# PRADUMAN-KR/Multimodal-Lip-Sync-Deepfake-Detection-System

Measured on NVIDIA B200. Metric: windows_per_sec, higher is better.
Workload: dtype bf16

## Files before the change

### multimodal-lip-sync-deepfake-detection-system_b200/csrc/bf16_path.cu

```cuda
#include "forward_common.h"
#include "tok_front.cuh"
#include "tok_fused.cuh"
#include "token_kernels.cuh"
#include "umma_conv.cuh"
#include "stem_ring.cuh"

#include <cuda_fp16.h>

#include <algorithm>
#include <array>
#include <cstdio>
#include <cstdlib>
#include <cstring>
#include <functional>

using namespace lsd;
using namespace lsdfw;

#define LSD_ENV(name) ([]() -> const char* { static const char* const v_ = getenv(name); return v_; }())

namespace {

uint16_t f2bf(float f) {
  uint32_t u;
// ... 653 lines not shown
        const long long cy = d[3] - d[2];
        cmin = std::min(cmin, cy); cmax = std::max(cmax, cy); csum += cy;
      }
      fprintf(stderr, "[sr] %d CTAs x %d steps: kernel span %.1f us (globaltimer), latest CTA start +%.1f us, CTA cycles min %lld avg %lld max %lld\n", nc,
              p.nsteps, (g1 - g0) / 1e3, smax / 1e3, cmin, csum / nc, cmax);
    }
    const long long t0 = hv[0];
    for (int k = 0; k < 32; ++k)
      fprintf(stderr, "[sr] step %2d | prod free %7lld issued %7lld | mma landed %7lld blockfree %7lld issued %7lld | epi complete %7lld back %7lld\n", k + 16,
              hv[(0 * 32 + k) * 2] - t0, hv[(0 * 32 + k) * 2 + 1] - t0, hv[(1 * 32 + k) * 2] - t0, hv[(1 * 32 + k) * 2 + 1] - t0,
              hv[(2 * 32 + k) * 2] - t0, hv[(3 * 32 + k) * 2] - t0, hv[(3 * 32 + k) * 2 + 1] - t0);
    h->prof.end(c.st);
    return 0;
  }
  launch_stem_ring(p, tab->grid, c.st);
  h->prof.end(c.st);
  return 0;
}

#define RUN(name, ...)                            \
  do {                                            \
    UArgs a_;                                     \
    __VA_ARGS__;                                  \
    if ((rc = run_umma(b, name, a_))) return rc;  \
  } while (0)

#define RUNC(ctx, name, ...)                        \
  do {                                              \
    UArgs a_;                                       \
    __VA_ARGS__;                                    \
    if ((rc = run_umma(ctx, name, a_))) return rc;  \
  } while (0)

#define RUNS(name, ...)                            \
  do {                                             \
    UArgs a_;                                      \
    __VA_ARGS__;                                   \
    if ((rc = run_umma(bs, name, a_))) return rc;  \
  } while (0)

PlanarOut pout(const BCtx& c, const PBuf& p, const PBuf* lo = nullptr, int plane_off = 0) {
  PlanarOut o;
  o.y = c.org(p) + (int64_t)plane_off * p.plane_stride;
  o.ylo = lo ? c.org(*lo) + (int64_t)plane_off * lo->plane_stride : nullptr;
  o.plane_stride = p.plane_stride;
  if (p.g.ow > 0 && p.g.HP == 1) { o.grp = p.g.W; o.grp_stride = p.g.RW; o.off = p.g.ow; }
  else { o.grp = 0; o.grp_stride = 0; o.off = 0; }
  return o;
}

int res_stage_umma(const BCtx& b, const std::string& p, const PBuf& x, const PBuf& mid, const PBuf& y, bool has_ds, int y_mode,
                   const PBuf* x_lo = nullptr, const PBuf* mid_lo = nullptr, const PBuf* y_lo = nullptr) {
  int rc = 0;
  RUN(p + ".conv1", a_.in = &x; a_.in_lo = x_lo; a_.og = mid.g; a_.act = ACT_RELU; a_.yp = &mid; a_.yp_lo = mid_lo);
  if (has_ds) RUN(p + ".conv2", a_.in = &mid; a_.in_lo = mid_lo; a_.in_ds = &x; a_.in_ds_lo = x_lo; a_.og = mid.g; a_.act = ACT_RELU;
                  a_.yp = &y; a_.yp_lo = y_lo; a_.y_mode = y_mode);
  else RUN(p + ".conv2", a_.in = &mid; a_.in_lo = mid_lo; a_.og = mid.g; a_.act = ACT_RELU; a_.yp = &y; a_.yp_lo = y_lo; a_.y_mode = y_mode;
           a_.res = &x; a_.res_lo = x_lo);
  return 0;
}

int run_umma_fold(const BCtx& c, const std::string& name, const PBuf& x, int Hi, int Wi, int stride, const PBuf* x_ds, int Hd, int Wd,
                  int Ho, int Wo, const PBuf& yp, int y_mode) {
  const auto itL = c.h->blayers.find(name + "#fold");
  if (itL == c.h->blayers.end()) return lsd_fail(c.h, LSD_ERR_UNSUPPORTED, "%s: no weights packed for the folded route (LSD_FOLD=0)", name.c_str());
  const BLayer& L = itL->second;
  const UcGeom& og = x.g;
  if (og.P_total >= ((int64_t)1 << 31) - 1024) return lsd_fail(c.h, LSD_ERR_SHAPE, "%s: more than 2^31 rows in one launch (reduce the batch)", name.c_str());
  if ((L.groups.size() == 2) != (x_ds != nullptr) || x.sets != Hi * Wi || (x_ds && x_ds->sets != Hd * Wd))
    return lsd_fail(c.h, LSD_ERR_ARG, "%s: folded inputs do not match the layer", name.c_str());
  UmmaConvP p;
  memset(&p, 0, sizeof(p));
  p.w = reinterpret_cast<const __nv_bfloat16*>(c.h->barena);
  p.bias = c.h->bbias + L.bias_off;
  p.Cout = L.ntile;
  p.act = ACT_RELU;
  p.g = og;
  p.fold = 1;
  p.y_mode = y_mode;
  p.y = c.org(yp);
  p.y_plane_stride = yp.plane_stride; p.y_set_stride = yp.set_stride;
  p.g2 = yp.g;
  p.ymap_W = Wo;
  int mt = 2;
  if (const char* e = LSD_ENV("LSD_FOLD_MT")) mt = std::max(1, std::min(4, atoi(e)));
  p.MT = (int)std::max<int64_t>(1, std::min<int64_t>(mt, (og.P_total + 127) / 128));
  p.nbuf = 1;
  p.issuers = std::min(p.MT, 4);
  uint32_t cols = 32;
  while ((int)cols < p.MT * L.ntile) cols *= 2;
  p.tmem_cols = cols;
  const int S = p.MT * 128;
  const PBuf* srcs[2] = {&x, x_ds};
  p.ngroups = (int)L.groups.size();
  p.nbands = p.ngroups;
  int max_a = 0, max_w = 0, min_k16 = 1 << 30;
  for (int gi = 0; gi < p.ngroups; ++gi) {
    const BGroup& G = L.groups[gi];
    UcGroup& ug = p.groups[gi];
    ug.band_begin = gi; ug.band_end = gi + 1;
    ug.k16 = G.k16; ug.taps_total = G.taps_total;
    ug.w_off = (int64_t)G.w_off; ug.slice_stride = (int64_t)G.slice_stride;
    UcBand& ub = p.bands[gi];
    const PBuf& src = *srcs[gi];
    ub.base = c.org(src);
    ub.plane_stride = src.plane_stride;
    ub.chunk_stride = 2 * src.plane_stride;
    ub.ntaps = gi == 0 ? 3 : 1;
    ub.start = gi == 0 ? -1 : 0;
    ub.len_extra = gi == 0 ? 2 : 0;
    for (int j = 0; j < ub.ntaps; ++j) ub.rel[j] = j;
    if ((int64_t)8 > src.origin) return lsd_fail(c.h, LSD_ERR_UNSUPPORTED, "%s: guard zone too small", name.c_str());
    max_a = std::max(max_a, 2 * (S + ub.len_extra) * 16);
    max_w = std::max(max_w, ub.ntaps * L.ntile * 32);
    min_k16 = std::min(min_k16, G.k16);
  }
  p.kpack = std::max(1, std::min(std::min(8, min_k16), (48 * 1024) / (max_a + max_w)));
  p.a_stage_bytes = ((uint32_t)(max_a * p.kpack) + 127u) & ~127u;
  p.w_stage_bytes = (uint32_t)(max_w * p.kpack);
  const int cslices = L.Cout / L.ntile;
  std::vector<std::array<int, 3>> pos;
  auto inb = [&](int o, int k, int n) { const int i = stride * o + k - 1; return i >= 0 && i < n; };
  for (int ho = 0; ho < Ho; ++ho)
    for (int wo = 0; wo < Wo; ++wo) {
      int nq = 0;
      for (int kh = 0; kh < 3; ++kh)
        for (int kw = 0; kw < 3; ++kw) nq += inb(ho, kh, Hi) && inb(wo, kw, Wi);
      pos.push_back({-nq, ho, wo});
    }
  std::stable_sort(pos.begin(), pos.end(), [](const std::array<int, 3>& a, const std::array<int, 3>& b) { return a[0] < b[0]; });
  const int nslices = (int)pos.size() * cslices;
  if (nslices > UC_MAX_FSLICES || Ho > 255 || Wo > 255) return lsd_fail(c.h, LSD_ERR_UNSUPPORTED, "%s: map too large for the folded route", name.c_str());
  auto chunks = [&](int k16) { return (k16 + p.kpack - 1) / p.kpack; };
  int off = 0;
  for (int i = 0; i < nslices; ++i) {
    const auto& q = pos[(size_t)(i / cslices)];
    const int nst = -q[0] * chunks(p.groups[0].k16) + (x_ds ? chunks(p.groups[1].k16) : 0);
    p.fslice[i] = UcFoldSlice{(uint16_t)off, (uint16_t)nst, (uint8_t)q[1], (uint8_t)q[2], (uint8_t)(i % cslices), 0};
    p.nst_tile = std::max(p.nst_tile, nst);
    off += nst;
  }
  if (off > 65535) return lsd_fail(c.h, LSD_ERR_UNSUPPORTED, "%s: folded stage programs too long", name.c_str());
  const uint32_t stage = p.a_stage_bytes + p.w_stage_bytes;
  const uint32_t prog_bytes = (uint32_t)p.nst_tile * (uint32_t)umma_conv_stage_desc_bytes();
  const uint32_t budget = 211u * 1024u - (uint32_t)umma_conv_extra_smem_bytes(p);
  if (prog_bytes + 2 * stage > budget) return lsd_fail(c.h, LSD_ERR_UNSUPPORTED, "%s: stage program of %u bytes does not fit", name.c_str(), prog_bytes);
  p.stages = std::max(2, std::min((int)((budget - prog_bytes) / stage), 8));
  if (const char* e = getenv("LSD_UMMA_SKIP")) p.skip = atoi(e);
  if (const char* why = umma_conv_config_error(p)) return lsd_fail(c.h, LSD_ERR_UNSUPPORTED, "%s: %s", name.c_str(), why);
  auto build = [&](std::vector<UcStageDesc>& v) {
    for (int i = 0; i < nslices; ++i) {
      const UcFoldSlice& f = p.fslice[i];
      for (int kh = 0; kh < 3; ++kh)
        for (int kw = 0; kw < 3; ++kw) {
          if (!inb(f.h, kh, Hi) || !inb(f.w, kw, Wi)) continue;
          UcBand bq = p.bands[0];
          bq.base = c.org(x) + (int64_t)((stride * f.h + kh - 1) * Wi + stride * f.w + kw - 1) * x.set_stride;
          bq.tap_begin = (kh * 3 + kw) * 3;
          for (int c0 = 0; c0 < p.groups[0].k16; c0 += p.kpack) v.push_back(umma_conv_stage(p, p.groups[0], bq, 0, c0, f.col));
        }
      if (x_ds) {
        UcBand bd = p.bands[1];
        bd.base = c.org(*x_ds) + (int64_t)(2 * f.h * Wd + 2 * f.w) * x_ds->set_stride;
        for (int c0 = 0; c0 < p.groups[1].k16; c0 += p.kpack) v.push_back(umma_conv_stage(p, p.groups[1], bd, 1, c0, f.col));
      }
    }
  };
  if (int rc = stage_program(c, name + "#fold", p, build, {(uint64_t)Hi, (uint64_t)Wi, (uint64_t)stride, (uint64_t)Hd, (uint64_t)Wd,
                                                          (uint64_t)x.set_stride, (uint64_t)(x_ds ? x_ds->set_stride : 0)})) return rc;
  double kflop = 0;
  for (const BGroup& G : L.groups) kflop += (double)G.taps_total * G.Cin;
  c.h->prof.begin(c.st, 2.0 * (double)og.N * og.T * Ho * Wo * L.Cout * kflop, 2);
  launch_umma_conv(p, nslices, c.st, c.h->num_sms, c.max_ctas);
  c.h->prof.end(c.st);
  return 0;
}

int res_stage_fold(const BCtx& b, const std::string& p, const PBuf& x, int Hi, int Wi, const PBuf& mid, int Ho, int Wo, const PBuf& y, int y_mode) {
  int rc = 0;
  if ((rc = run_umma_fold(b, p + ".conv1", x, Hi, Wi, 2, nullptr, 0, 0, Ho, Wo, mid, UC_Y_FOLD))) return rc;
  return run_umma_fold(b, p + ".conv2", mid, Ho, Wo, 1, &x, Hi, Wi, Ho, Wo, y, y_mode);
}

}

static int pack_tok_fused(lsd_handle* h, const std::vector<float>& f32) {
  std::vector<TfBlock> blocks;
  tf_layer_blocks(blocks);
  std::vector<uint32_t> stage_bytes;
  for (const TfBlock& b : blocks)
    for (int k0 = 0; k0 < b.k16; k0 += b.kps) stage_bytes.push_back((uint32_t)b.kps * (uint32_t)b.N * 32u);
  std::vector<__half> w;
  std::vector<float> vec((size_t)TF_LAYERS * TF_VEC_LAYER + (size_t)(2 * TF_LAYERS + 1) * TF_D, 0.f);
  std::vector<float> cum(TF_D, 0.f);
  float* cum_out = vec.data() + (size_t)TF_LAYERS * TF_VEC_LAYER;
  for (int l = 0; l < TF_LAYERS; ++l) {
    const std::string k = "t" + std::to_string(l);
    const ConvP &cin = h->convs.at(k + ".in"), &cout = h->convs.at(k + ".out"), &cf1 = h->convs.at(k + ".ff1"), &cf2 = h->convs.at(k + ".ff2");
    const size_t w0 = w.size();
    for (const TfBlock& b : blocks) {
      const ConvP& c = b.kind == 0 ? cin : (b.kind == 1 ? cout : (b.kind == 2 ? cf1 : cf2));
      for (int k16 = 0; k16 < b.k16; ++k16)
        for (int pl = 0; pl < 2; ++pl)
          for (int n = 0; n < b.N; ++n)
            for (int e = 0; e < 8; ++e) {
              const int kk = k16 * 16 + pl * 8 + e;
              int co, ci;
              if (b.kind == 0) { co = ((n % 96) / 32) * 256 + (2 * b.idx + n / 96) * 32 + (n % 32); ci = kk; }
              else if (b.kind == 1) { co = n; ci = 64 * b.idx + kk; }
              else if (b.kind == 2) { co = 128 * b.idx + n; ci = kk; }
              else { co = n; ci = 128 * b.idx + kk; }
              w.push_back(__float2half_rn(f32[c.w_off + (size_t)ci * c.Cout + co]));
            }
    }
    if (l == 0) h->tokf_layer_bytes = (uint32_t)((w.size() - w0) * sizeof(__half));
    float* lv = vec.data() + (size_t)l * TF_VEC_LAYER;
    const char* names[4] = {".ln1.w", ".ln1.b", ".ln2.w", ".ln2.b"};
    for (int i = 0; i < 4; ++i) memcpy(lv + 256 * i, &f32[h->vecs.at(k + names[i])], 256 * sizeof(float));
    for (int n = 0; n < 768; ++n) {
      const int hp = n / 192, r = n % 192;
      lv[1024 + n] = f32[cin.shift_off + ((r % 96) / 32) * 256 + (2 * hp + r / 96) * 32 + (r % 32)];
    }
    memcpy(lv + 1024 + 768, &f32[cf1.shift_off], 1024 * sizeof(float));
    memcpy(cum_out + (size_t)(2 * l) * TF_D, cum.data(), TF_D * sizeof(float));
    for (int i = 0; i < TF_D; ++i) cum[i] += f32[cout.shift_off + i];
    memcpy(cum_out + (size_t)(2 * l + 1) * TF_D, cum.data(), TF_D * sizeof(float));
    for (int i = 0; i < TF_D; ++i) cum[i] += f32[cf2.shift_off + i];
  }
  memcpy(cum_out + (size_t)(2 * TF_LAYERS) * TF_D, cum.data(), TF_D * sizeof(float));
  h->tokf_n_stage = (int)stage_bytes.size();
  for (void* q : {(void*)h->tokf_w, (void*)h->tokf_stage_bytes, (void*)h->tokf_vec}) if (q) cudaFree(q);
  h->tokf_w = nullptr; h->tokf_stage_bytes = nullptr; h->tokf_vec = nullptr;
  cudaError_t e = cudaMalloc(&h->tokf_w, w.size() * sizeof(__half));
  if (e == cudaSuccess) e = cudaMemcpy(h->tokf_w, w.data(), w.size() * sizeof(__half), cudaMemcpyHostToDevice);
  if (e == cudaSuccess) e = cudaMalloc(&h->tokf_stage_bytes, stage_bytes.size() * sizeof(uint32_t));
  if (e == cudaSuccess) e = cudaMemcpy(h->tokf_stage_bytes, stage_bytes.data(), stage_bytes.size() * sizeof(uint32_t), cudaMemcpyHostToDevice);
  if (e == cudaSuccess) e = cudaMalloc(&h->tokf_vec, vec.size() * sizeof(float));
  if (e == cudaSuccess) e = cudaMemcpy(h->tokf_vec, vec.data(), vec.size() * sizeof(float), cudaMemcpyHostToDevice);
  if (e != cudaSuccess) return lsd_fail(h, LSD_ERR_CUDA, "pack_tok_fused: %s", cudaGetErrorString(e));
  return 0;
}

static int pack_tok_front(lsd_handle* h, const std::vector<float>& f32) {
  std::vector<__half> w;
  w.reserve((size_t)TFR_K16_TOTAL * 16 * 256);
  auto emit = [&](int k16, auto&& get) {
    for (int k = 0; k < k16; ++k)
      for (int pl = 0; pl < 2; ++pl)
        for (int n = 0; n < 256; ++n)
          for (int e = 0; e < 8; ++e) w.push_back(__float2half_rn(get(k * 16 + pl * 8 + e, n)));
  };
  const ConvP &o0 = h->convs.at("cross.v2a.out"), &o1 = h->convs.at("cross.a2v.out"), &g0 = h->convs.at("cross.gate0"),
// ... 732 lines not shown
```

### multimodal-lip-sync-deepfake-detection-system_b200/csrc/umma_conv.cu

```cuda
#include "umma_conv.cuh"
#include "token_kernels.cuh"

#include <algorithm>
#include <cstdio>
#include <cstdlib>
#include <cstring>

#include "lsd_kernels.h"
#include "umma.cuh"

namespace lsd {

using namespace umma;

struct F8 { float v[8]; };
__device__ __noinline__ F8 gelu8(F8 x) {
#pragma unroll
  for (int e = 0; e < 8; ++e) x.v[e] = 0.5f * x.v[e] * (1.0f + erff(x.v[e] * 0.70710678118654752f));
  return x;
}

__device__ __forceinline__ float uc_act(float v, int act) {
  if (act == ACT_RELU) return fmaxf(v, 0.0f);
  if (act == ACT_GELU) return 0.5f * v * (1.0f + erff(v * 0.70710678118654752f));
// ... 334 lines not shown
              for (int q = 0; q < 4; ++q) pre[4 + q] = *reinterpret_cast<const uint4*>(p.res_lo + roff + (int64_t)q * p.res_plane_stride);
            }
          } else if (use_r32) {
#pragma unroll
            for (int q = 0; q < 8; ++q) pre[q] = *reinterpret_cast<const uint4*>(r32row + c0 + 4 * q);
          }
          tmem_ld_wait();
#pragma unroll
          for (int q = 0; q < 4; ++q) {
            const int c = c0 + 8 * q;
            F8 x;
#pragma unroll
            for (int e = 0; e < 8; ++e) x.v[e] = v[8 * q + e];
            if (valid) {
              const float4 b0 = *reinterpret_cast<const float4*>(&bias_s[c]);
              const float4 b1 = *reinterpret_cast<const float4*>(&bias_s[c + 4]);
              x.v[0] += b0.x; x.v[1] += b0.y; x.v[2] += b0.z; x.v[3] += b0.w; x.v[4] += b1.x; x.v[5] += b1.y; x.v[6] += b1.z; x.v[7] += b1.w;
              if (use_res) {
                float f[8];
                unpack8(pre[q], f);
#pragma unroll
                for (int e = 0; e < 8; ++e) x.v[e] += f[e];
                if (use_lo) {
                  unpack8(pre[4 + q], f);
#pragma unroll
                  for (int e = 0; e < 8; ++e) x.v[e] += f[e];
                }
              } else if (use_r32) {
                const uint4 q0 = pre[2 * q], q1 = pre[2 * q + 1];
                x.v[0] += __uint_as_float(q0.x); x.v[1] += __uint_as_float(q0.y); x.v[2] += __uint_as_float(q0.z); x.v[3] += __uint_as_float(q0.w);
                x.v[4] += __uint_as_float(q1.x); x.v[5] += __uint_as_float(q1.y); x.v[6] += __uint_as_float(q1.z); x.v[7] += __uint_as_float(q1.w);
              }
              if (p.act == ACT_GELU) {
                x = gelu8(x);
              } else {
#pragma unroll
                for (int e = 0; e < 8; ++e) x.v[e] = fmaxf(x.v[e], act_lo);
              }
              if (y32row) {
                float4* o = reinterpret_cast<float4*>(y32row + c);
                o[0] = make_float4(x.v[0], x.v[1], x.v[2], x.v[3]);
                o[1] = make_float4(x.v[4], x.v[5], x.v[6], x.v[7]);
              }
            } else {
#pragma unroll
              for (int e = 0; e < 8; ++e) x.v[e] = 0.0f;
            }
            if (store_planar) {
              const uint4 hi4 = pack8(x.v);
              const int64_t off = (int64_t)((ch0 + c) >> 3) * p.y_plane_stride + dst;
              *reinterpret_cast<uint4*>(p.y + off) = hi4;
              if (p.ylo) {
                float hf[8];
                unpack8(hi4, hf);
#pragma unroll
                for (int e = 0; e < 8; ++e) hf[e] = x.v[e] - hf[e];
                *reinterpret_cast<uint4*>(p.ylo + off) = pack8(hf);
              }
            }
          }
        }
        }
      }
      tc_fence_before();
      __syncwarp();
      if (lane == 0) {
        if (CTA2 && cta_rank != 0) mbar_arrive_cluster(mapa_shared(smem_u32(&tempty2_bar[buf]), 0u));
        else mbar_arrive(&tempty_bar[buf]);
      }
      if (dbg && warp == UC_EPI_WARP0 && lane == 0 && lt == 0) p.dbg[5] = clock64();
    }
  }
done:
  tc_fence_before();
  if constexpr (CTA2) cluster_sync_all();
  else __syncthreads();
  if (warp == UC_EPI_WARP0) {
    if constexpr (CTA2) tmem_dealloc2(tmem_base, p.tmem_cols);
    else tmem_dealloc(tmem_base, p.tmem_cols);
  }
  if (dbg && tid == 0) { p.dbg[6] = clock64(); p.dbg[7] = num_tiles; }
}

UcStageDesc umma_conv_stage(const UmmaConvP& p, const UcGroup& g, const UcBand& bd, int band, int c0, int col) {
  const int S = p.MT * 128;
  const int bcols = p.cta2 ? p.Cout / 2 : p.Cout;
  const int nc = std::min(p.kpack, g.k16 - c0);
  UcStageDesc d;
  const uint32_t bytesW = (uint32_t)bd.ntaps * (uint32_t)bcols * 32u;
  d.bytesA = bd.toeplitz ? (uint32_t)(S + bd.len_extra + 1 + 2 * (nc - 1)) * 16u : (uint32_t)(S + bd.len_extra) * 16u;
  uint32_t n_a = bd.toeplitz ? 1u : 2u * (uint32_t)nc;
  const bool w_merged = bd.ntaps == g.taps_total;
  uint32_t n_w = w_merged ? 1u : (uint32_t)nc;
  d.w_copy_bytes = w_merged ? (uint32_t)nc * bytesW : bytesW;
  d.w_dst_step = bytesW;
  if (p.skip & 1) n_a = 0;
  if (p.skip & 2) n_w = 0;
  d.tx_bytes = n_a * d.bytesA + (n_w ? (uint32_t)nc * bytesW : 0u);
  d.a_src = reinterpret_cast<uint64_t>(bd.base + (int64_t)c0 * bd.chunk_stride + (int64_t)bd.start * 8);
  d.chunk_stride_b = (uint64_t)bd.chunk_stride * 2u;
  d.plane_stride_b = (uint64_t)bd.plane_stride * 2u;
  d.w_src = reinterpret_cast<uint64_t>(p.w + g.w_off + (col > 0 ? (int64_t)col * g.slice_stride : 0) +
                                       ((int64_t)c0 * g.taps_total + bd.tap_begin) * (int64_t)bcols * 16);
  d.w_slice_stride_b = col >= 0 ? 0u : (uint64_t)g.slice_stride * 2u;
  d.w_src_step = (uint32_t)g.taps_total * (uint32_t)bcols * 32u;
  d.counts = n_a | (n_w << 8) | ((uint32_t)band << 16) | ((uint32_t)nc << 24);
  return d;
}

void umma_conv_build_program(const UmmaConvP& p, UcStageDesc* out) {
  int s = 0;
  for (int gi = 0; gi < p.ngroups; ++gi) {
    const UcGroup& g = p.groups[gi];
    for (int c0 = 0; c0 < g.k16; c0 += p.kpack)
      for (int b = g.band_begin; b < g.band_end; ++b) out[s++] = umma_conv_stage(p, g, p.bands[b], b, c0);
  }
}

size_t umma_conv_smem_bytes(const UmmaConvP& p) {
  size_t b = (size_t)p.stages * (p.a_stage_bytes + p.w_stage_bytes) + (size_t)p.nst_tile * sizeof(UcStageDesc) + 1024;
  return b + umma_conv_extra_smem_bytes(p);
}
int umma_conv_stage_desc_bytes() { return (int)sizeof(UcStageDesc); }
static bool uc_is_generic(const UmmaConvP& p);
size_t umma_conv_extra_smem_bytes(const UmmaConvP& p) {
  if (uc_is_generic(p)) return 0;
  return 128 + 2048 + (size_t)(p.cta2 ? p.Cout / 2 : p.Cout) * 32u;
}

static bool uc_is_generic(const UmmaConvP& p) {
  return p.y32 || p.res32 || p.ylo || p.res_lo || p.act == ACT_GELU || p.y_mode == UC_Y_NONE || (p.Cout & 31);
}
const char* umma_conv_config_error(const UmmaConvP& p) {
  if (2 * p.kpack + p.kpack > 32) return "K chunks per stage exceed the producer lanes";
  if (p.res && p.res32) return "bf16 and fp32 residuals are mutually exclusive";
  if (uc_is_generic(p) && (p.Cout & 63)) return "the generic epilogue needs a column slice that is a multiple of 64";
  if (p.MT / p.issuers > 4 || p.MT % p.issuers) return "unsupported M-tiles per issuing warp";
  if (p.fold && (uc_is_generic(p) || p.cta2 || p.res || p.MT > 4))
    return "folded convolutions need the lean epilogue, no residual, single CTAs and at most 4 M-tiles";
  if (p.cta2 && (uc_is_generic(p) || (p.Cout & 31))) return "CTA pairs need the lean epilogue and a multiple of 32 columns";
  return nullptr;
}

cudaError_t umma_conv_device_init() {
  cudaError_t e = cudaFuncSetAttribute(umma_conv_kernel<0>, cudaFuncAttributeMaxDynamicSharedMemorySize, 223 * 1024);
  if (e == cudaSuccess) e = cudaFuncSetAttribute(umma_conv_kernel<1>, cudaFuncAttributeMaxDynamicSharedMemorySize, 223 * 1024);
  if (e == cudaSuccess) e = cudaFuncSetAttribute(umma_conv_kernel<3>, cudaFuncAttributeMaxDynamicSharedMemorySize, 223 * 1024);
  if (e == cudaSuccess) e = video_rows_device_init();
  return e;
}

void launch_umma_conv(const UmmaConvP& p, int n_slices, cudaStream_t s, int num_sms, int max_ctas) {
  if (const char* why = umma_conv_config_error(p)) { fprintf(stderr, "umma_conv: %s\n", why); abort(); }
  const int S = p.MT * 128;
  const int tiles = (int)((p.g.P_total + S - 1) / S);
  const int budget = (max_ctas > 0 && max_ctas < num_sms) ? max_ctas : num_sms;
  int gx = (budget + n_slices - 1) / n_slices;
  gx = gx < 1 ? 1 : (gx > tiles ? tiles : gx);
  const bool generic = uc_is_generic(p);
  if (p.cta2) {
    if (n_slices != 1) { fprintf(stderr, "umma_conv: CTA pairs take one column slice\n"); abort(); }
    const int pairs = (tiles + 1) / 2;
    int gp = budget / 2;
    gp = gp < 1 ? 1 : (gp > pairs ? pairs : gp);
    cudaLaunchConfig_t cfg = {};
    cfg.gridDim = dim3(2 * gp, 1, 1);
    cfg.blockDim = dim3(UC_THREADS, 1, 1);
    cfg.dynamicSmemBytes = umma_conv_smem_bytes(p);
    cfg.stream = s;
    cudaLaunchAttribute at[1];
    at[0].id = cudaLaunchAttributeClusterDimension;
    at[0].val.clusterDim.x = 2; at[0].val.clusterDim.y = 1; at[0].val.clusterDim.z = 1;
    cfg.attrs = at; cfg.numAttrs = 1;
    cudaLaunchKernelEx(&cfg, umma_conv_kernel<3>, p);
    count_launch();
    return;
  }
  if (p.fold) gx = tiles;
  if (generic) umma_conv_kernel<1><<<dim3(gx, n_slices), UC_THREADS, umma_conv_smem_bytes(p), s>>>(p);
  else umma_conv_kernel<0><<<dim3(gx, n_slices), UC_THREADS, umma_conv_smem_bytes(p), s>>>(p);
  count_launch();
}

__global__ void pack_planar_kernel(const float* __restrict__ x, __nv_bfloat16* __restrict__ y, int64_t plane_stride, int64_t set_stride,
                                   UcGeom g, UcGeom g2, int C, int parity, int64_t total) {
  const int64_t i = (int64_t)blockIdx.x * blockDim.x + threadIdx.x;
  if (i >= total) return;
  const int64_t npos = (int64_t)g.N * g.T * g.H * g.W;
  const int chunk = (int)(i / npos);
  int64_t r = i - (int64_t)chunk * npos;
  const int w = (int)(r % g.W); r /= g.W;
  const int h = (int)(r % g.H); r /= g.H;
  const int t = (int)(r % g.T);
  const int n = (int)(r / g.T);
  const float* src = x + ((((int64_t)n * g.T + t) * g.H + h) * g.W + w) * C + chunk * 8;
  float v[8];
#pragma unroll
  for (int e = 0; e < 8; ++e) v[e] = src[e];
  int64_t dst;
  if (parity) dst = (int64_t)((h & 1) * 2 + (w & 1)) * set_stride + uc_flat(g2, n, t, h >> 1, w >> 1) * 8;
  else dst = uc_flat(g, n, t, h, w) * 8;
  *reinterpret_cast<uint4*>(y + (int64_t)chunk * plane_stride + dst) = pack8(v);
}
void launch_pack_planar(const float* x, __nv_bfloat16* y, int64_t plane_stride, int64_t set_stride, UcGeom g, UcGeom g2, int C,
                        int parity, cudaStream_t s) {
  const int64_t total = (int64_t)g.N * g.T * g.H * g.W * (C / 8);
  if (total == 0) return;
  pack_planar_kernel<<<(unsigned)((total + 255) / 256), 256, 0, s>>>(x, y, plane_stride, set_stride, g, g2, C, parity, total);
  count_launch();
}

__global__ void unpack_planar_kernel(const __nv_bfloat16* __restrict__ x, int64_t plane_stride, UcGeom g, int C, float* __restrict__ y,
                                     int ld, int64_t total) {
  const int64_t i = (int64_t)blockIdx.x * blockDim.x + threadIdx.x;
  if (i >= total) return;
  const int nch = C / 8;
  const int chunk = (int)(i % nch);
  int64_t r = i / nch;
  const int64_t row = r;
  const int w = (int)(r % g.W); r /= g.W;
  const int h = (int)(r % g.H); r /= g.H;
  const int t = (int)(r % g.T);
  const int n = (int)(r / g.T);
  const uint4 v = *reinterpret_cast<const uint4*>(x + (int64_t)chunk * plane_stride + uc_flat(g, n, t, h, w) * 8);
  float f[8];
  unpack8(v, f);
  float4* o = reinterpret_cast<float4*>(y + row * ld + chunk * 8);
  o[0] = make_float4(f[0], f[1], f[2], f[3]);
  o[1] = make_float4(f[4], f[5], f[6], f[7]);
}
void launch_unpack_planar(const __nv_bfloat16* x, int64_t plane_stride, UcGeom g, int C, float* y, int ld, cudaStream_t s) {
  const int64_t total = (int64_t)g.N * g.T * g.H * g.W * (C / 8);
  if (total == 0) return;
  unpack_planar_kernel<<<(unsigned)((total + 255) / 256), 256, 0, s>>>(x, plane_stride, g, C, y, ld, total);
  count_launch();
}

__global__ void unpack_planar_any_kernel(const __nv_bfloat16* __restrict__ x, const __nv_bfloat16* __restrict__ xlo, int64_t plane_stride,
                                         int64_t set_stride, UcGeom g, int C, int sets, int Hf, int Wf, float* __restrict__ y, int64_t total) {
  const int64_t i = (int64_t)blockIdx.x * blockDim.x + threadIdx.x;
  if (i >= total) return;
  const int nch = C / 8;
  const int chunk = (int)(i % nch);
  int64_t r = i / nch;
  const int64_t row = r;
  const int w = (int)(r % Wf); r /= Wf;
  const int h = (int)(r % Hf); r /= Hf;
  const int t = (int)(r % g.T);
  const int n = (int)(r / g.T);
  int64_t src;
  if (sets == 1) src = uc_flat(g, n, t, h, w) * 8;
  else if (g.SL == 1 && sets == Hf * Wf) src = (int64_t)(h * Wf + w) * set_stride + uc_flat(g, n, t, 0, 0) * 8;
  else if (Wf == g.W) src = (int64_t)((h & 1) * 2) * set_stride + uc_flat(g, n, t, h >> 1, w) * 8;
  else src = (int64_t)((h & 1) * 2 + (w & 1)) * set_stride + uc_flat(g, n, t, h >> 1, w >> 1) * 8;
  src += (int64_t)chunk * plane_stride;
  float f[8];
  unpack8(*reinterpret_cast<const uint4*>(x + src), f);
  if (xlo) {
    float fl[8];
    unpack8(*reinterpret_cast<const uint4*>(xlo + src), fl);
// ... 678 lines not shown
```

### multimodal-lip-sync-deepfake-detection-system_b200/csrc/umma_conv.cuh

```cuda
#pragma once
#include <cuda_bf16.h>
#include <cuda_runtime.h>
#include <stdint.h>

namespace lsd {

constexpr int UC_MAX_BANDS = 16;
constexpr int UC_MAX_TAPS = 12;
constexpr int UC_MAX_GROUPS = 6;

struct UcBand {
  const __nv_bfloat16* base;
  int64_t plane_stride;
  int64_t chunk_stride;
  int start;
  int len_extra;
  int ntaps;
  int tap_begin;
  int toeplitz;
  int rel[UC_MAX_TAPS];
};

struct UcGroup {
  int band_begin, band_end;
  int k16;
  int taps_total;
  int64_t w_off;
  int64_t slice_stride;
};

enum UcOut { UC_Y_NONE = 0, UC_Y_PLAIN = 1, UC_Y_PARITY = 2, UC_Y_PARITY_H = 3, UC_Y_FOLD = 5, UC_Y_MAP = 6 };

constexpr int UC_MAX_FSLICES = 96;
struct UcFoldSlice {
  uint16_t prog_off, nst;
  uint8_t h, w;
  uint8_t col, pad_;
};

struct UcGeom {
  int N, T, H, W;
  int TS, ot, HP, oh, RW, ow, SL;
  int64_t P_total;
  uint32_t mSL, mRW, mTS;
  int sSL, sRW, sTS;
};

inline void uc_magic(uint32_t d, uint32_t& m, int& s) {
  s = 0;
  while (((uint64_t)1 << s) < d) ++s;
  m = (uint32_t)((((uint64_t)1 << (31 + s)) / d) + 1);
}

struct alignas(16) UcStageDesc {
  uint64_t a_src;
  uint64_t w_src;
  uint64_t chunk_stride_b;
  uint64_t plane_stride_b;
  uint64_t w_slice_stride_b;
  uint32_t bytesA;
  uint32_t w_copy_bytes;
  uint32_t w_dst_step;
  uint32_t w_src_step;
  uint32_t tx_bytes;
  uint32_t counts;
};
static_assert(sizeof(UcStageDesc) == 64, "UcStageDesc must be 64 bytes");

struct UmmaConvP {
  const __nv_bfloat16* w;
  const float* bias;
  const __nv_bfloat16* res;
  const __nv_bfloat16* res_lo;
  int64_t res_plane_stride;
  const float* res32;
  int res32_ld;
  __nv_bfloat16* y;
  __nv_bfloat16* ylo;
  int64_t y_plane_stride, y_set_stride;
  int y_mode;
  float* y32;
  int y32_ld;
  int y32_outer_stride, y32_row_off;
  int act;
  int Cout;
  int MT, stages, ngroups, nbands;
  int issuers;
  int nbuf;
  long long* dbg;
  const UcStageDesc* prog;
  int nst_tile;
  int skip;
  int kpack;
  uint32_t a_stage_bytes, w_stage_bytes, tmem_cols;
  int cta2;
  UcGeom g;
  UcGeom g2;
  UcGroup groups[UC_MAX_GROUPS];
  UcBand bands[UC_MAX_BANDS];
  int ymap_W;
  int fold;
  UcFoldSlice fslice[UC_MAX_FSLICES];
};

size_t umma_conv_smem_bytes(const UmmaConvP& p);
int umma_conv_stage_desc_bytes();
size_t umma_conv_extra_smem_bytes(const UmmaConvP& p);
void umma_conv_build_program(const UmmaConvP& p, UcStageDesc* out);
UcStageDesc umma_conv_stage(const UmmaConvP& p, const UcGroup& g, const UcBand& bd, int band, int c0, int col = -1);
const char* umma_conv_config_error(const UmmaConvP& p);
void launch_umma_conv(const UmmaConvP& p, int n_slices, cudaStream_t s, int num_sms, int max_ctas = 0);
cudaError_t umma_conv_device_init();
cudaError_t video_rows_device_init();

void launch_pack_planar(const float* x, __nv_bfloat16* y, int64_t plane_stride, int64_t set_stride, UcGeom g, UcGeom g2, int C,
                        int parity, cudaStream_t s);
void launch_unpack_planar(const __nv_bfloat16* x, int64_t plane_stride, UcGeom g, int C, float* y, int ld, cudaStream_t s);
void launch_unpack_planar_any(const __nv_bfloat16* x, const __nv_bfloat16* xlo, int64_t plane_stride, int64_t set_stride, UcGeom g, int C, int sets,
                              int Hf, int Wf, float* y, cudaStream_t s);
void launch_planar_mean(const __nv_bfloat16* x, int64_t plane_stride, UcGeom g, int C, float* y, int ld, int per_window, cudaStream_t s);
void launch_planar_delta(const __nv_bfloat16* x, int64_t x_plane_stride, UcGeom g, __nv_bfloat16* d, int64_t d_plane_stride, UcGeom gd,
                         int C, cudaStream_t s);
void launch_planar_maxpool(const __nv_bfloat16* x, int64_t x_plane_stride, UcGeom gi, __nv_bfloat16* y, int64_t y_plane_stride, UcGeom go,
                           int C, cudaStream_t s, const __nv_bfloat16* xlo = nullptr, __nv_bfloat16* ylo = nullptr);

void launch_video_rows(const void* video, int dtype, int layout, const float* lapw, const float* lapw_host, __nv_bfloat16* xs, __nv_bfloat16* xl,
                       int64_t set_stride, UcGeom g, int H, int W, cudaStream_t s, int num_sms, const int32_t* starts = nullptr, int n_frames = 0);
bool video_rows_bulk_ok(const void* video, int dtype, int layout, int W);

inline UcGeom make_geom_ex(int N, int T, int H, int W, int tpad, int oh, int hp_extra, int ow, int wp_extra) {
  UcGeom g;
  g.N = N; g.T = T; g.H = H; g.W = W;
  g.TS = T + tpad; g.ot = tpad;
  g.HP = H + oh + hp_extra; g.oh = oh;
  g.RW = W + ow + wp_extra; g.ow = ow;
  g.SL = g.HP * g.RW;
  g.P_total = ((int64_t)N * g.TS + tpad) * g.SL;
  uc_magic((uint32_t)g.SL, g.mSL, g.sSL);
  uc_magic((uint32_t)g.RW, g.mRW, g.sRW);
  uc_magic((uint32_t)g.TS, g.mTS, g.sTS);
  return g;
}
inline UcGeom make_geom(int N, int T, int H, int W) { return make_geom_ex(N, T, H, W, 1, 1, 0, 1, 0); }
inline UcGeom make_geom_rows(int rows) { return make_geom_ex(1, 1, 1, rows, 0, 0, 0, 0, 0); }

}
```

Before: 25880.

## Add persistent work-claiming walk kernel for folded UMMA convolutions

Adds a persistent kernel for the folded residual-stage convolutions. It runs a host-built list of (slice, tile-range) jobs sorted largest first, claimed through an atomic counter, with a double-buffered TMEM accumulator so the epilogue of one tile overlaps the MMAs of the next. The M-tile count is reduced when too few jobs would exist per SM, and bias rows for all column slices are preloaded into shared memory. This targets poor load balance and idle tensor cores between tiles in the previous one-CTA-per-(tile,slice) grid, at the cost of atomic claiming, more TMEM columns, and a more complex barrier protocol.

Result: no change. 25640 (median of 6 runs) (-0.9%).

```diff
diff --git a/multimodal-lip-sync-deepfake-detection-system_b200/csrc/bf16_path.cu b/multimodal-lip-sync-deepfake-detection-system_b200/csrc/bf16_path.cu
--- a/multimodal-lip-sync-deepfake-detection-system_b200/csrc/bf16_path.cu
+++ b/multimodal-lip-sync-deepfake-detection-system_b200/csrc/bf16_path.cu
@@ -759,13 +759,22 @@
   p.y_plane_stride = yp.plane_stride; p.y_set_stride = yp.set_stride;
   p.g2 = yp.g;
   p.ymap_W = Wo;
+  static const bool walk = !(LSD_ENV("LSD_FOLD_WALK") && atoi(LSD_ENV("LSD_FOLD_WALK")) == 0);
+  static const bool claim = !(LSD_ENV("LSD_FOLD_CLAIM") && atoi(LSD_ENV("LSD_FOLD_CLAIM")) == 0);
   int mt = 2;
   if (const char* e = LSD_ENV("LSD_FOLD_MT")) mt = std::max(1, std::min(4, atoi(e)));
+  const int ctas = (c.max_ctas > 0 && c.max_ctas < c.h->num_sms) ? c.max_ctas : c.h->num_sms;
+  if (walk) {
+    mt = std::min(mt, std::max(1, 256 / L.ntile));
+    const int64_t nsl = (int64_t)Ho * Wo * (L.Cout / L.ntile);
+    while (mt > 1 && nsl * ((og.P_total + mt * 128 - 1) / (mt * 128)) < 4 * (int64_t)ctas) mt /= 2;
+  }
   p.MT = (int)std::max<int64_t>(1, std::min<int64_t>(mt, (og.P_total + 127) / 128));
-  p.nbuf = 1;
+  p.fold = walk ? 2 : 1;
+  p.nbuf = walk ? 2 : 1;
   p.issuers = std::min(p.MT, 4);
   uint32_t cols = 32;
-  while ((int)cols < p.MT * L.ntile) cols *= 2;
+  while ((int)cols < p.nbuf * p.MT * L.ntile) cols *= 2;
   p.tmem_cols = cols;
   const int S = p.MT * 128;
   const PBuf* srcs[2] = {&x, x_ds};
@@ -796,28 +805,21 @@
   p.a_stage_bytes = ((uint32_t)(max_a * p.kpack) + 127u) & ~127u;
   p.w_stage_bytes = (uint32_t)(max_w * p.kpack);
   const int cslices = L.Cout / L.ntile;
-  std::vector<std::array<int, 3>> pos;
-  auto inb = [&](int o, int k, int n) { const int i = stride * o + k - 1; return i >= 0 && i < n; };
-  for (int ho = 0; ho < Ho; ++ho)
-    for (int wo = 0; wo < Wo; ++wo) {
-      int nq = 0;
-      for (int kh = 0; kh < 3; ++kh)
-        for (int kw = 0; kw < 3; ++kw) nq += inb(ho, kh, Hi) && inb(wo, kw, Wi);
-      pos.push_back({-nq, ho, wo});
-    }
-  std::stable_sort(pos.begin(), pos.end(), [](const std::array<int, 3>& a, const std::array<int, 3>& b) { return a[0] < b[0]; });
-  const int nslices = (int)pos.size() * cslices;
-  if (nslices > UC_MAX_FSLICES || Ho > 255 || Wo > 255) return lsd_fail(c.h, LSD_ERR_UNSUPPORTED, "%s: map too large for the folded route", name.c_str());
   auto chunks = [&](int k16) { return (k16 + p.kpack - 1) / p.kpack; };
-  int off = 0;
-  for (int i = 0; i < nslices; ++i) {
-    const auto& q = pos[(size_t)(i / cslices)];
-    const int nst = -q[0] * chunks(p.groups[0].k16) + (x_ds ? chunks(p.groups[1].k16) : 0);
-    p.fslice[i] = UcFoldSlice{(uint16_t)off, (uint16_t)nst, (uint8_t)q[1], (uint8_t)q[2], (uint8_t)(i % cslices), 0};
-    p.nst_tile = std::max(p.nst_tile, nst);
-    off += nst;
-  }
-  if (off > 65535) return lsd_fail(c.h, LSD_ERR_UNSUPPORTED, "%s: folded stage programs too long", name.c_str());
+  const std::vector<UcFoldSliceH> sl = uc_fold_slices(Hi, Wi, stride, Ho, Wo, cslices, chunks(p.groups[0].k16), x_ds ? chunks(p.groups[1].k16) : 0);
+  const int nslices = (int)sl.size();
+  const int prog_len = nslices ? sl.back().prog_off + sl.back().nst : 0;
+  for (const UcFoldSliceH& f : sl) p.nst_tile = std::max(p.nst_tile, f.nst);
+  if (!walk) {
+    if (nslices > UC_MAX_FSLICES || Ho > 255 || Wo > 255) return lsd_fail(c.h, LSD_ERR_UNSUPPORTED, "%s: map too large for the folded route", name.c_str());
+    if (prog_len > 65535) return lsd_fail(c.h, LSD_ERR_UNSUPPORTED, "%s: folded stage programs too long", name.c_str());
+    for (int i = 0; i < nslices; ++i)
+      p.fslice[i] = UcFoldSlice{(uint16_t)sl[i].prog_off, (uint16_t)sl[i].nst, (uint8_t)sl[i].h, (uint8_t)sl[i].w, (uint8_t)sl[i].col, 0};
+  }
+  const int tiles = (int)((og.P_total + S - 1) / S);
+  const int tiles_per_job = walk ? std::max(1, (int)(((int64_t)nslices * tiles) / (4 * ctas))) : 0;
+  const std::vector<UcFoldJob> jobs = walk ? uc_fold_jobs(sl, tiles, tiles_per_job) : std::vector<UcFoldJob>();
+  if (walk) { p.nst_tile = 0; p.fold_ncol = cslices; }
   const uint32_t stage = p.a_stage_bytes + p.w_stage_bytes;
   const uint32_t prog_bytes = (uint32_t)p.nst_tile * (uint32_t)umma_conv_stage_desc_bytes();
   const uint32_t budget = 211u * 1024u - (uint32_t)umma_conv_extra_smem_bytes(p);
@@ -825,9 +827,10 @@
   p.stages = std::max(2, std::min((int)((budget - prog_bytes) / stage), 8));
   if (const char* e = getenv("LSD_UMMA_SKIP")) p.skip = atoi(e);
   if (const char* why = umma_conv_config_error(p)) return lsd_fail(c.h, LSD_ERR_UNSUPPORTED, "%s: %s", name.c_str(), why);
+  const int job_units = (int)((jobs.size() * sizeof(UcFoldJob) + sizeof(UcStageDesc) - 1) / sizeof(UcStageDesc));
   auto build = [&](std::vector<UcStageDesc>& v) {
-    for (int i = 0; i < nslices; ++i) {
-      const UcFoldSlice& f = p.fslice[i];
+    auto inb = [&](int o, int k, int n) { const int i = stride * o + k - 1; return i >= 0 && i < n; };
+    for (const UcFoldSliceH& f : sl) {
       for (int kh = 0; kh < 3; ++kh)
         for (int kw = 0; kw < 3; ++kw) {
           if (!inb(f.h, kh, Hi) || !inb(f.w, kw, Wi)) continue;
@@ -842,9 +845,21 @@
         for (int c0 = 0; c0 < p.groups[1].k16; c0 += p.kpack) v.push_back(umma_conv_stage(p, p.groups[1], bd, 1, c0, f.col));
       }
     }
+    if (walk) {
+      v.resize((size_t)prog_len + job_units + 1);
+      memset(v.data() + prog_len, 0, ((size_t)job_units + 1) * sizeof(UcStageDesc));
+      memcpy(v.data() + prog_len, jobs.data(), jobs.size() * sizeof(UcFoldJob));
+    }
   };
   if (int rc = stage_program(c, name + "#fold", p, build, {(uint64_t)Hi, (uint64_t)Wi, (uint64_t)stride, (uint64_t)Hd, (uint64_t)Wd,
-                                                          (uint64_t)x.set_stride, (uint64_t)(x_ds ? x_ds->set_stride : 0)})) return rc;
+                                                          (uint64_t)x.set_stride, (uint64_t)(x_ds ? x_ds->set_stride : 0),
+                                                          (uint64_t)Ho, (uint64_t)tiles_per_job})) return rc;
+  if (walk) {
+    p.fjobs = reinterpret_cast<const UcFoldJob*>(p.prog + prog_len);
+    p.fclaim = const_cast<int*>(reinterpret_cast<const int*>(p.prog + prog_len + job_units));
+    p.njobs = (int)jobs.size();
+    p.fold_claim = claim ? 1 : 0;
+  }
   double kflop = 0;
   for (const BGroup& G : L.groups) kflop += (double)G.taps_total * G.Cin;
   c.h->prof.begin(c.st, 2.0 * (double)og.N * og.T * Ho * Wo * L.Cout * kflop, 2);
diff --git a/multimodal-lip-sync-deepfake-detection-system_b200/csrc/umma_conv.cu b/multimodal-lip-sync-deepfake-detection-system_b200/csrc/umma_conv.cu
--- a/multimodal-lip-sync-deepfake-detection-system_b200/csrc/umma_conv.cu
+++ b/multimodal-lip-sync-deepfake-detection-system_b200/csrc/umma_conv.cu
@@ -440,6 +440,244 @@
   if (dbg && tid == 0) { p.dbg[6] = clock64(); p.dbg[7] = num_tiles; }
 }
 
+constexpr int UC_JOB_SLOTS = 4;
+__device__ __forceinline__ UcFoldJob uc_load_job(const UcFoldJob* jobs, int j) {
+  UcFoldJob r;
+  const uint4* s = reinterpret_cast<const uint4*>(jobs + j);
+  reinterpret_cast<uint4*>(&r)[0] = __ldg(s);
+  reinterpret_cast<uint4*>(&r)[1] = __ldg(s + 1);
+  return r;
+}
+__global__ void __launch_bounds__(UC_THREADS, 1) umma_fold_walk_kernel(const __grid_constant__ UmmaConvP p) {
+  extern __shared__ __align__(1024) uint8_t smem[];
+  __shared__ uint64_t full_bar[8], empty_bar[8], tfull_bar[2], tempty_bar[2], jfull_bar[UC_JOB_SLOTS], jempty_bar[UC_JOB_SLOTS];
+  __shared__ uint64_t jwant_bar;
+  __shared__ int job_s[UC_JOB_SLOTS];
+  __shared__ uint32_t tmem_base_s;
+  const int tid = threadIdx.x, warp = tid >> 5, lane = tid & 31;
+  const int S = p.MT * 128;
+  const uint32_t stage_bytes = p.a_stage_bytes + p.w_stage_bytes;
+  const uint32_t buf_cols = (uint32_t)(p.MT * p.Cout);
+  const int n_issuers = p.issuers;
+  const int npw = min(UC_PROD_WARPS, p.stages);
+  if (tid == 0) {
+    for (int i = 0; i < p.stages; ++i) { mbar_init(&full_bar[i], 1); mbar_init(&empty_bar[i], n_issuers); }
+    for (int i = 0; i < 2; ++i) { mbar_init(&tfull_bar[i], n_issuers); mbar_init(&tempty_bar[i], UC_EPI_WARPS); }
+    for (int i = 0; i < UC_JOB_SLOTS; ++i) { mbar_init(&jfull_bar[i], 1); mbar_init(&jempty_bar[i], npw + n_issuers + UC_EPI_WARPS); }
+    mbar_init(&jwant_bar, 1);
+    fence_barrier_init();
+  }
+  if (warp == UC_EPI_WARP0) { tmem_alloc(&tmem_base_s, p.tmem_cols); tmem_relinquish(); }
+  uint8_t* const bias_a = smem + (size_t)p.stages * stage_bytes;
+  uint8_t* const bias_b = bias_a + 2048;
+  for (int i = tid; i < 128; i += UC_THREADS) reinterpret_cast<uint4*>(bias_a)[i] = make_uint4(0x3F803F80u, 0x00003F80u, 0u, 0u);
+  for (int i = tid; i < 2 * p.Cout * p.fold_ncol; i += UC_THREADS) {
+    const int c = i / (2 * p.Cout), k = i - c * 2 * p.Cout;
+    uint4 o = make_uint4(0u, 0u, 0u, 0u);
+    if (k < p.Cout && p.bias) {
+      const float b = p.bias[c * p.Cout + k];
+      const __nv_bfloat16 hi = __float2bfloat16_rn(b);
+      const float r1 = b - __bfloat162float(hi);
+      const __nv_bfloat16 mid = __float2bfloat16_rn(r1);
+      const __nv_bfloat16 lo = __float2bfloat16_rn(r1 - __bfloat162float(mid));
+      o.x = (uint32_t)__bfloat16_as_ushort(hi) | ((uint32_t)__bfloat16_as_ushort(mid) << 16);
+      o.y = (uint32_t)__bfloat16_as_ushort(lo);
+    }
+    reinterpret_cast<uint4*>(bias_b)[i] = o;
+  }
+  fence_proxy_async_smem();
+  tc_fence_before();
+  __syncthreads();
+  tc_fence_after();
+  const uint32_t tmem_base = tmem_base_s;
+  auto next_job = [&](int i) -> int {
+    const int s = i % UC_JOB_SLOTS;
+    mbar_wait(&jfull_bar[s], (uint32_t)(i / UC_JOB_SLOTS) & 1u);
+    const int j = job_s[s];
+    __syncwarp();
+    if (lane == 0 && j >= 0) mbar_arrive(&jempty_bar[s]);
+    return j;
+  };
+
+  if (warp < UC_PROD_WARPS) {
+    if (warp >= npw) goto done;
+    const uint32_t smem_base = smem_u32(smem);
+    int k = 0;
+    for (int i = 0;; ++i) {
+      const int j = next_job(i);
+      if (j < 0) break;
+      const UcFoldJob jb = uc_load_job(p.fjobs, j);
+      const uint4* prog = reinterpret_cast<const uint4*>(p.prog + jb.prog_off);
+      for (int tile = jb.tile0; tile < jb.tile1; ++tile, k += jb.nst) {
+        const uint64_t p0_bytes = (uint64_t)tile * (uint64_t)S * 16u;
+        for (int si = ((warp - k) % npw + npw) % npw; si < jb.nst; si += npw) {
+          const int kk = k + si;
+          const int stage = kk % p.stages;
+          const uint32_t ph = (uint32_t)(kk / p.stages) & 1u;
+          UcStageDesc d;
+#pragma unroll
+          for (int q = 0; q < 4; ++q) reinterpret_cast<uint4*>(&d)[q] = __ldg(prog + 4 * si + q);
+          const uint32_t counts = d.counts;
+          const uint32_t n_a = counts & 0xffu, n_all = n_a + ((counts >> 8) & 0xffu);
+          const bool is_a = (uint32_t)lane < n_a;
+          const bool mine = (uint32_t)lane < n_all;
+          const uint32_t jc = is_a ? ((uint32_t)lane >> 1) : ((uint32_t)lane - n_a);
+          const uint32_t sa = smem_base + (uint32_t)stage * stage_bytes;
+          const uint64_t gsrc = is_a ? d.a_src + p0_bytes + (uint64_t)jc * d.chunk_stride_b + (uint64_t)(lane & 1) * d.plane_stride_b
+                                     : d.w_src + (uint64_t)jc * (uint64_t)d.w_src_step;
+          const uint32_t dst = is_a ? sa + (uint32_t)lane * d.bytesA : sa + p.a_stage_bytes + jc * d.w_dst_step;
+          const uint32_t nbytes = is_a ? d.bytesA : d.w_copy_bytes;
+          mbar_wait(&empty_bar[stage], ph ^ 1u);
+          if (lane == 0) mbar_arrive_expect_tx(&full_bar[stage], d.tx_bytes);
+          __syncwarp();
+          if (mine) bulk_s2(dst, reinterpret_cast<const void*>(gsrc), nbytes, &full_bar[stage]);
+          __syncwarp();
+          if (lane == 0 && tile == jb.tile1 - 1 && si == max(0, jb.nst - p.stages)) mbar_arrive(&jwant_bar);
+        }
+      }
+    }
+  } else if (warp < UC_MMA_WARP0 + UC_MMA_WARPS) {
+    if (warp == UC_MMA_WARP0 + UC_MMA_WARPS - 1) {
+      for (int i = 0;; ++i) {
+        const int s = i % UC_JOB_SLOTS;
+        if (i > 0) mbar_wait(&jwant_bar, (uint32_t)(i - 1) & 1u);
+        mbar_wait(&jempty_bar[s], ((uint32_t)(i / UC_JOB_SLOTS) & 1u) ^ 1u);
+        int j = 0;
+        if (lane == 0) {
+          if (p.fold_claim) {
+            j = atomicAdd(p.fclaim, 1);
+            if (j >= p.njobs) {
+              if (j == p.njobs + (int)gridDim.x - 1) atomicExch(p.fclaim, 0);
+              j = -1;
+            }
+          } else {
+            j = (int)blockIdx.x + i * (int)gridDim.x;
+            if (j >= p.njobs) j = -1;
+          }
+          job_s[s] = j;
+          mbar_arrive(&jfull_bar[s]);
+        }
+        if (__shfl_sync(0xffffffffu, j, 0) < 0) break;
+      }
+      goto done;
+    }
+    if (warp - UC_MMA_WARP0 >= n_issuers) goto done;
+    const int warp_u = __shfl_sync(0xffffffffu, warp, 0);
+    const int mt_n = p.MT / n_issuers;
+    const int mt_lo = (warp_u - UC_MMA_WARP0) * mt_n;
+    const uint32_t idesc = idesc_bf16(128, p.Cout);
+    const uint32_t smem_base = smem_u32(smem);
+    const uint64_t desc_hi64 = ((uint64_t)8 << 32) | ((uint64_t)1 << 46);
+    const uint32_t b_lbo = (uint32_t)p.Cout << 16;
+    const uint32_t tap_w = (uint32_t)p.Cout * 2u;
+    const uint32_t leader = elect_one() ? 1u : 0u;
+    const int ch_main = (p.groups[0].k16 + p.kpack - 1) / p.kpack;
+    const int st_ds = p.ngroups == 2 ? (p.groups[1].k16 + p.kpack - 1) / p.kpack : 0;
+    const uint64_t da_bias = desc_hi64 | (uint64_t)(smem_u32(bias_a) >> 4);
+    int stage = 0, lt = 0;
+    uint32_t ph = 0;
+    for (int i = 0;; ++i) {
+      const int j = next_job(i);
+      if (j < 0) break;
+      const UcFoldJob jb = uc_load_job(p.fjobs, j);
+      const int nst = __shfl_sync(0xffffffffu, jb.nst, 0);
+      const int nmain = nst - st_ds;
+      const int tile1 = __shfl_sync(0xffffffffu, jb.tile1, 0);
+      const uint64_t db_bias = desc_hi64 | (uint64_t)(((smem_u32(bias_b) + (uint32_t)__shfl_sync(0xffffffffu, jb.col, 0) * (uint32_t)p.Cout * 32u) >> 4) | b_lbo);
+      for (int tile = jb.tile0; tile < tile1; ++tile, ++lt) {
+        const int buf = lt & 1;
+        const uint32_t use = (uint32_t)lt >> 1;
+        const uint32_t tb = tmem_base + (uint32_t)buf * buf_cols + (uint32_t)(mt_lo * p.Cout);
+        mbar_wait(&tempty_bar[buf], (use & 1u) ^ 1u);
+        tc_fence_after();
+        mma_bf16_ss_pred(tb, da_bias, db_bias, idesc, 0u, leader);
+        if (mt_n > 1) mma_bf16_ss_pred(tb + (uint32_t)p.Cout, da_bias, db_bias, idesc, 0u, leader);
+        int cb = 0;
+        for (int si = 0; si < nst; ++si) {
+          const int b = si < nmain ? 0 : 1;
+          if (si == nmain) cb = 0;
+          const int nc = min(p.kpack, p.groups[b].k16 - cb * p.kpack);
+          cb = (b == 0 && cb + 1 == ch_main) ? 0 : cb + 1;
+          const UcBand& bd = p.bands[b];
+          const int ntaps = bd.ntaps;
+          const uint32_t unitsA = (uint32_t)(S + bd.len_extra);
+          const uint32_t a_lbo = unitsA << 16;
+          const uint32_t a_chunk = 2u * unitsA;
+          const uint32_t w_chunk = (uint32_t)ntaps * tap_w;
+          mbar_wait(&full_bar[stage], ph);
+          tc_fence_after();
+          const uint32_t sa = ((smem_base + (uint32_t)stage * stage_bytes) >> 4) + (uint32_t)mt_lo * 128u;
+          const uint32_t sw = ((smem_base + (uint32_t)stage * stage_bytes + p.a_stage_bytes) >> 4) | b_lbo;
+          for (int jc = 0; jc < nc; ++jc) {
+            const uint32_t aj = (sa + (uint32_t)jc * a_chunk) | a_lbo;
+            uint32_t wj = sw + (uint32_t)jc * w_chunk;
+#pragma unroll 1
+            for (int tp = 0; tp < ntaps; ++tp) {
+              const uint64_t da = desc_hi64 | (uint64_t)(aj + (uint32_t)bd.rel[tp]), db = desc_hi64 | (uint64_t)wj;
+              mma_bf16_ss_pred(tb, da, db, idesc, 1u, leader);
+              if (mt_n > 1) mma_bf16_ss_pred(tb + (uint32_t)p.Cout, da + 128u, db, idesc, 1u, leader);
+              wj += tap_w;
+            }
+          }
+          mma_commit_pred(&empty_bar[stage], leader);
+          if (++stage == p.stages) { stage = 0; ph ^= 1u; }
+        }
+        mma_commit_pred(&tfull_bar[buf], leader);
+      }
+    }
+  } else {
+    const int quarter = warp & 3;
+    const int half = (warp - UC_EPI_WARP0) >> 2;
+    const int rowt = quarter * 32 + lane;
+    const bool split_m = p.MT >= 2;
+    const bool split_c = !split_m && (p.Cout & 63) == 0;
+    const int m_end = (!split_m && !split_c && half == 1) ? 0 : p.MT;
+    const int cbeg = split_c ? half * (p.Cout >> 1) : 0, cend = split_c ? cbeg + (p.Cout >> 1) : p.Cout;
+    const int64_t yps = p.y_plane_stride * 2;
+    int lt = 0;
+    for (int i = 0;; ++i) {
+      const int j = next_job(i);
+      if (j < 0) break;
+      const UcFoldJob jb = uc_load_job(p.fjobs, j);
+      char* const ybase = reinterpret_cast<char*>(p.y + (int64_t)((jb.col * p.Cout + cbeg) >> 3) * p.y_plane_stride);
+      for (int tile = jb.tile0; tile < jb.tile1; ++tile, ++lt) {
+        const int buf = lt & 1;
+        const uint32_t use = (uint32_t)lt >> 1;
+        const uint32_t tb = tmem_base + (uint32_t)buf * buf_cols + ((uint32_t)(quarter * 32) << 16);
+        mbar_wait(&tfull_bar[buf], use & 1u);
+        tc_fence_after();
+        for (int m = split_m ? half : 0; m < m_end; m += split_m ? 2 : 1) {
+          const int64_t P = (int64_t)tile * S + (int64_t)m * 128 + rowt;
+          int n = 0, t = 0, h = 0, w = 0;
+          const bool valid = uc_decode(p.g, P, n, t, h, w);
+          const int64_t dst = p.y_mode == UC_Y_FOLD ? (int64_t)(jb.h * p.ymap_W + jb.w) * p.y_set_stride + uc_flat(p.g2, n, t, 0, 0) * 8
+                                                    : uc_flat(p.g2, n, t, jb.h, jb.w) * 8;
+          const bool store = valid && !(p.skip & 4);
+          char* yp = ybase + dst * 2;
+          uint32_t ta = tb + (uint32_t)(m * p.Cout + cbeg);
+#pragma unroll 1
+          for (int c = cbeg; c < cend; c += 32, yp += 4 * yps, ta += 32) {
+            float v[32];
+            tmem_ld32(ta, v);
+            tmem_ld_wait();
+            if (store) {
+#pragma unroll
+              for (int q = 0; q < 4; ++q) *reinterpret_cast<uint4*>(yp + q * yps) = pack8_relu(v + 8 * q);
+            }
+          }
+        }
+        tc_fence_before();
+        __syncwarp();
+        if (lane == 0) mbar_arrive(&tempty_bar[buf]);
+      }
+    }
+  }
+done:
+  tc_fence_before();
+  __syncthreads();
+  if (warp == UC_EPI_WARP0) tmem_dealloc(tmem_base, p.tmem_cols);
+}
+
 UcStageDesc umma_conv_stage(const UmmaConvP& p, const UcGroup& g, const UcBand& bd, int band, int c0, int col) {
   const int S = p.MT * 128;
   const int bcols = p.cta2 ? p.Cout / 2 : p.Cout;
@@ -483,6 +721,7 @@
 static bool uc_is_generic(const UmmaConvP& p);
 size_t umma_conv_extra_smem_bytes(const UmmaConvP& p) {
   if (uc_is_generic(p)) return 0;
+  if (p.fold == 2) return 128 + 2048 + (size_t)p.fold_ncol * p.Cout * 32u;
   return 128 + 2048 + (size_t)(p.cta2 ? p.Cout / 2 : p.Cout) * 32u;
 }
 
@@ -496,6 +735,9 @@
   if (p.MT / p.issuers > 4 || p.MT % p.issuers) return "unsupported M-tiles per issuing warp";
   if (p.fold && (uc_is_generic(p) || p.cta2 || p.res || p.MT > 4))
     return "folded convolutions need the lean epilogue, no residual, single CTAs and at most 4 M-tiles";
+  if (p.fold == 2 && (p.issuers > UC_MMA_WARPS - 1 || p.nbuf != 2 || 2 * p.MT * p.Cout > (int)p.tmem_cols || p.tmem_cols > 512 ||
+                      p.act != ACT_RELU || (p.y_mode != UC_Y_FOLD && p.y_mode != UC_Y_MAP) || p.stages > 8 || p.fold_ncol < 1))
+    return "the persistent folded walk needs two accumulator buffers, a spare MMA warp, ReLU and a folded / map destination";
   if (p.cta2 && (uc_is_generic(p) || (p.Cout & 31))) return "CTA pairs need the lean epilogue and a multiple of 32 columns";
   return nullptr;
 }
@@ -504,6 +746,7 @@
   cudaError_t e = cudaFuncSetAttribute(umma_conv_kernel<0>, cudaFuncAttributeMaxDynamicSharedMemorySize, 223 * 1024);
   if (e == cudaSuccess) e = cudaFuncSetAttribute(umma_conv_kernel<1>, cudaFuncAttributeMaxDynamicSharedMemorySize, 223 * 1024);
   if (e == cudaSuccess) e = cudaFuncSetAttribute(umma_conv_kernel<3>, cudaFuncAttributeMaxDynamicSharedMemorySize, 223 * 1024);
+  if (e == cudaSuccess) e = cudaFuncSetAttribute(umma_fold_walk_kernel, cudaFuncAttributeMaxDynamicSharedMemorySize, 223 * 1024);
   if (e == cudaSuccess) e = video_rows_device_init();
   return e;
 }
@@ -534,6 +777,11 @@
     count_launch();
     return;
   }
+  if (p.fold == 2) {
+    umma_fold_walk_kernel<<<std::max(1, std::min(budget, p.njobs)), UC_THREADS, umma_conv_smem_bytes(p), s>>>(p);
+    count_launch();
+    return;
+  }
   if (p.fold) gx = tiles;
   if (generic) umma_conv_kernel<1><<<dim3(gx, n_slices), UC_THREADS, umma_conv_smem_bytes(p), s>>>(p);
   else umma_conv_kernel<0><<<dim3(gx, n_slices), UC_THREADS, umma_conv_smem_bytes(p), s>>>(p);
diff --git a/multimodal-lip-sync-deepfake-detection-system_b200/csrc/umma_conv.cuh b/multimodal-lip-sync-deepfake-detection-system_b200/csrc/umma_conv.cuh
--- a/multimodal-lip-sync-deepfake-detection-system_b200/csrc/umma_conv.cuh
+++ b/multimodal-lip-sync-deepfake-detection-system_b200/csrc/umma_conv.cuh
@@ -2,6 +2,9 @@
 #include <cuda_bf16.h>
 #include <cuda_runtime.h>
 #include <stdint.h>
+
+#include <algorithm>
+#include <vector>
 
 namespace lsd {
 
@@ -37,6 +40,47 @@
   uint8_t h, w;
   uint8_t col, pad_;
 };
+struct alignas(16) UcFoldJob {
+  int32_t prog_off, nst;
+  int32_t h, w, col;
+  int32_t tile0, tile1;
+  int32_t pad_;
+};
+static_assert(sizeof(UcFoldJob) == 32, "UcFoldJob is loaded as two 16-byte words");
+
+struct UcFoldSliceH { int h, w, col, nq, nst, prog_off; };
+inline std::vector<UcFoldSliceH> uc_fold_slices(int Hi, int Wi, int stride, int Ho, int Wo, int cslices, int st_main, int st_ds) {
+  std::vector<UcFoldSliceH> pos;
+  auto inb = [&](int o, int k, int n) { const int i = stride * o + k - 1; return i >= 0 && i < n; };
+  for (int ho = 0; ho < Ho; ++ho)
+    for (int wo = 0; wo < Wo; ++wo) {
+      int nq = 0;
+      for (int kh = 0; kh < 3; ++kh)
+        for (int kw = 0; kw < 3; ++kw) nq += inb(ho, kh, Hi) && inb(wo, kw, Wi);
+      pos.push_back({ho, wo, 0, nq, nq * st_main + st_ds, 0});
+    }
+  std::stable_sort(pos.begin(), pos.end(), [](const UcFoldSliceH& a, const UcFoldSliceH& b) { return a.nq > b.nq; });
+  std::vector<UcFoldSliceH> out;
+  int off = 0;
+  for (const UcFoldSliceH& q : pos)
+    for (int c = 0; c < cslices; ++c) {
+      UcFoldSliceH s = q;
+      s.col = c; s.prog_off = off;
+      off += s.nst;
+      out.push_back(s);
+    }
+  return out;
+}
+inline std::vector<UcFoldJob> uc_fold_jobs(const std::vector<UcFoldSliceH>& slices, int tiles, int tiles_per_job) {
+  std::vector<UcFoldJob> jobs;
+  for (const UcFoldSliceH& s : slices)
+    for (int t0 = 0; t0 < tiles; t0 += tiles_per_job)
+      jobs.push_back(UcFoldJob{s.prog_off, s.nst, s.h, s.w, s.col, t0, std::min(tiles, t0 + tiles_per_job), 0});
+  std::stable_sort(jobs.begin(), jobs.end(), [](const UcFoldJob& a, const UcFoldJob& b) {
+    return (int64_t)a.nst * (a.tile1 - a.tile0) > (int64_t)b.nst * (b.tile1 - b.tile0);
+  });
+  return jobs;
+}
 
 struct UcGeom {
   int N, T, H, W;
@@ -101,6 +145,9 @@
   int ymap_W;
   int fold;
   UcFoldSlice fslice[UC_MAX_FSLICES];
+  const UcFoldJob* fjobs;
+  int* fclaim;
+  int njobs, fold_ncol, fold_claim, pad_walk_;
 };
 
 size_t umma_conv_smem_bytes(const UmmaConvP& p);
```
